# toprakdeviren/gpu-bpe

Hardware: AMD Instinct MI355X
Metric: BPE merges/sec + tokenize GB/s, 1 GiB UTF-8 @ 32K vocab, 1/2/4/8 MI355X (higher is better)
Workload: dtype u16; 1 GPU; headline: 32K-vocab BPE train on 1,073,741,824 B English-like UTF-8 (seed 2, 0.5% 3-byte punctuation), heuristic word boundaries, reference compaction; step = one complete training run (trainer creation + all 32,512 merges) on the HBM-resident corpus; train_bytes=1073741824, target_vocab=32768, parallelism=single

## Files before the change

gpu-bpe_amd/csrc/common.h:

```cpp
#pragma once

#include <hip/hip_runtime.h>
#include <cstdint>
#include <cstdio>
#include <cstdlib>
#include <cstring>
#include <map>
#include <mutex>
#include <string>
#include <type_traits>
#include <unordered_map>
#include <utility>
#include <vector>

#include "../../include/gpubpe.h"

struct GbpePool {
    std::multimap<uint64_t, void*> idle;
    std::unordered_map<void*, uint64_t> busy;
    uint64_t idle_bytes = 0, hits = 0, misses = 0;
};

struct GbpeGrowBuf {
    void* p = nullptr;
// ... 68 lines not shown
        if (p && cap >= n) return hipSuccess;
        GbpeArray nb;
        hipError_t e = nb.reserve(c, n, esz);
        if (e == hipSuccess && p && keep) e = hipMemcpyAsync(nb.p, p, keep * esz, hipMemcpyDeviceToDevice, s);
        if (e == hipSuccess) e = hipStreamSynchronize(s);
        if (e == hipSuccess) *this = std::move(nb);
        return e;
    }
};

int gbpe_set_error(gbpe_ctx* ctx, int code, const char* fmt, ...);

#define GBPE_HIP(ctx, call)                                                              \
    do {                                                                                 \
        hipError_t _e = (call);                                                          \
        if (_e != hipSuccess)                                                            \
            return gbpe_set_error((ctx), _e == hipErrorOutOfMemory ? GBPE_E_OOM           \
                                                                   : GBPE_E_DEVICE,      \
                                  "%s failed: %s (%s:%d)", #call, hipGetErrorString(_e), \
                                  __FILE__, __LINE__);                                   \
    } while (0)

#define GBPE_LAUNCH_CHECK(ctx) GBPE_HIP(ctx, hipGetLastError())

__device__ __forceinline__ uint32_t gbpe_fmix32(uint32_t x) {
    x = (x ^ (x >> 16)) * 0x7feb352du;
    x = (x ^ (x >> 15)) * 0x846ca68bu;
    return x ^ (x >> 16);
}

__host__ __device__ static inline uint64_t gbpe_div_up(uint64_t a, uint64_t b) { return (a + b - 1) / b; }

constexpr const char* kGbpeDebugKeys[] = {
    "lexicon", "lex_check", "rehash", "delta_mt", "zt", "rfl", "rflz", "lxwg", "lxtwo", "pair", "pseg", "prej", "zsmax", "zs32", "poison",
    "encode_slice", "decode_slice", "dec_plain", "me_cs", "htime", "ptrace", "rtime",
};

inline long gbpe_debug_knob(const char* key, long def) {
    const char* e = getenv("GBPE_DEBUG");
    if (!e) return def;
    const size_t kl = strlen(key);
    for (const char* p = e; *p;) {
        if (!strncmp(p, key, kl) && p[kl] == '=') return strtol(p + kl + 1, nullptr, 10);
        const char* c = strchr(p, ',');
        if (!c) break;
        p = c + 1;
    }
    return def;
}

inline std::string gbpe_debug_unknown() {
    const char* e = getenv("GBPE_DEBUG");
    for (const char* p = e ? e : ""; *p;) {
        const size_t el = strcspn(p, ","), kl = strcspn(p, ",=");
        bool ok = el == 0;
        for (const char* k : kGbpeDebugKeys) ok = ok || (kl < el && strlen(k) == kl && !strncmp(p, k, kl));
        if (!ok) return std::string(p, kl ? kl : el);
        p += el + (p[el] == ',');
    }
    return "";
}

int gbpe_pretok_gpt4_launch(gbpe_ctx* ctx, const uint8_t* d_bytes, uint64_t n, uint8_t* d_ws);
int gbpe_pretok_gpt4_docs_launch(gbpe_ctx* ctx, const uint8_t* d_bytes, uint64_t n, const uint8_t* d_flags, uint8_t* d_ws);
int gbpe_pretok_cl100k_launch(gbpe_ctx* ctx, const uint8_t* d_bytes, uint64_t n, const uint8_t* d_flags, uint8_t* d_ws);
int gbpe_pretok_o200k_launch(gbpe_ctx* ctx, const uint8_t* d_bytes, uint64_t n, const uint8_t* d_flags, uint8_t* d_ws);
constexpr uint32_t GBPE_DOC_BAD_ORDER = 1u, GBPE_DOC_BAD_FIRST = 2u, GBPE_DOC_BAD_LAST = 4u;
// ... 9 lines not shown
```

gpu-bpe_amd/csrc/lexicon.h:

```cpp

constexpr uint32_t LX_LIT = 0x80000000u;
constexpr uint32_t LX_LONG = 0x40000000u;
constexpr uint32_t LX_LMAX = 64;
constexpr int LX_WPT = 16;
constexpr int LX_LT = 2048;
constexpr uint32_t LX_PROBES = 4096;

template <typename S>
__device__ __forceinline__ bool lx_is_start(uint32_t prev, uint32_t cur, bool first) {
    return first || (cur & Sym<S>::WS) || !(cur & Sym<S>::TM) || !(prev & Sym<S>::TM);
}

template <typename S>
__global__ __launch_bounds__(TPB) void k_lx_count(const S* __restrict__ x, uint32_t len, uint32_t* __restrict__ tilecnt) {
    __shared__ uint32_t s[TPB / 64];
    const uint64_t base = (uint64_t)blockIdx.x * TILE;
    uint32_t c = 0;
#pragma unroll 4
    for (int k = 0; k < EPT; ++k) {
        const uint64_t i = base + (uint64_t)k * TPB + threadIdx.x;
        if (i < len) c += lx_is_start<S>(i ? (uint32_t)x[i - 1] : 0u, (uint32_t)x[i], i == 0) ? 1u : 0u;
    }
    c = wave_sum_u32(c);
    if ((threadIdx.x & 63) == 0) s[threadIdx.x >> 6] = c;
    __syncthreads();
    if (threadIdx.x == 0) {
        uint32_t t = 0;
        for (int w = 0; w < TPB / 64; ++w) t += s[w];
        tilecnt[blockIdx.x] = t;
    }
}

template <typename S>
__global__ __launch_bounds__(TPB) void k_lx_wpos(const S* __restrict__ x, uint32_t len, const uint32_t* __restrict__ tpre,
                                                 const uint64_t* __restrict__ tblk, uint32_t* __restrict__ wpos) {
    __shared__ uint32_t pre[EPT * (TPB / 64)];
    const int lane = threadIdx.x & 63, wid = threadIdx.x >> 6;
    const uint64_t base = (uint64_t)blockIdx.x * TILE;
    uint32_t f = 0;
#pragma unroll 4
    for (int k = 0; k < EPT; ++k) {
        const uint64_t i = base + (uint64_t)k * TPB + threadIdx.x;
        const bool st = i < len && lx_is_start<S>(i ? (uint32_t)x[i - 1] : 0u, (uint32_t)x[i], i == 0);
        f |= (st ? 1u : 0u) << k;
        const unsigned long long m = __ballot(st);
        if (lane == 0) pre[k * (TPB / 64) + wid] = (uint32_t)__popcll(m);
    }
    __syncthreads();
    if (threadIdx.x == 0) {
        uint32_t run = tpre[blockIdx.x] + (uint32_t)tblk[blockIdx.x / SCAN_BLK];
        for (int q = 0; q < EPT * (TPB / 64); ++q) {
            const uint32_t v = pre[q];
            pre[q] = run;
            run += v;
        }
    }
    __syncthreads();
    const unsigned long long lt = (1ull << lane) - 1ull;
    for (int k = 0; k < EPT; ++k) {
        const bool st = (f >> k) & 1u;
        const unsigned long long m = __ballot(st);
        if (st) wpos[pre[k * (TPB / 64) + wid] + (uint32_t)__popcll(m & lt)] = (uint32_t)(base + (uint64_t)k * TPB + threadIdx.x);
    }
}

template <typename S>
__device__ __forceinline__ unsigned long long lx_hash(const S* __restrict__ x, uint32_t s, uint32_t L) {
    unsigned long long h = 0x9E3779B97F4A7C15ull ^ (unsigned long long)L;
    for (uint32_t i0 = 0; i0 < L; i0 += 8) {
        uint32_t v[8];
#pragma unroll
        for (int k = 0; k < 8; ++k) v[k] = i0 + k < L ? (uint32_t)x[s + i0 + k] : 0u;
#pragma unroll
        for (int k = 0; k < 8; ++k) {
            if (i0 + k >= L) break;
            h ^= (unsigned long long)v[k];
            h *= 0x100000001B3ull;
            h ^= h >> 29;
        }
    }
    h ^= h >> 33;
    h *= 0xff51afd7ed558ccdull;
    h ^= h >> 33;
    h *= 0xc4ceb9fe1a85ec53ull;
    h ^= h >> 33;
    return h ? h : 1ull;
}

__device__ __forceinline__ uint32_t lx_home(unsigned long long h, uint32_t mask) { return (uint32_t)(h ^ (h >> 32)) & mask; }

struct alignas(16) LxSlot {
    unsigned long long key;
    uint32_t rep;
    uint32_t cnt;
};

__device__ __forceinline__ uint32_t lx_slice(uint32_t P) { return P >= (1u << 20) ? P >> 8 : (P < 4096u ? P : 4096u); }
__device__ __forceinline__ uint32_t lx_next(uint32_t slot, uint32_t sm) { return (slot & ~sm) | ((slot + 1u) & sm); }
__device__ __forceinline__ uint32_t lx_bucket(unsigned long long h, uint32_t P) {
    return lx_home(h, P - 1) / lx_slice(P);
}

__device__ bool lx_insert(LxSlot* __restrict__ wt, uint32_t P, unsigned long long h, uint32_t rep, uint32_t c,
                          uint32_t maxp = LX_PROBES) {
    const uint32_t sm = lx_slice(P) - 1u;
    uint32_t slot = lx_home(h, P - 1);
    if (maxp > sm + 1u) maxp = sm + 1u;
    for (uint32_t p = 0; p < maxp; ++p, slot = lx_next(slot, sm)) {
        unsigned long long k = wt[slot].key;
        if (k == 0ull) {
            k = atomicCAS(&wt[slot].key, 0ull, h);
            if (k == 0ull) {
                wt[slot].rep = rep;
                atomicAdd(&wt[slot].cnt, c);
                return true;
            }
        }
        if (k == h) {
            atomicAdd(&wt[slot].cnt, c);
            return true;
        }
    }
    return false;
}

__device__ uint4 lx_find(const LxSlot* __restrict__ wt, uint32_t P, unsigned long long h) {
    const uint32_t sm = lx_slice(P) - 1u;
    uint32_t slot = lx_home(h, P - 1);
    for (uint32_t p = 0; p <= sm && p < LX_PROBES; ++p, slot = lx_next(slot, sm)) {
        const uint4 v = *reinterpret_cast<const uint4*>(&wt[slot]);
        const unsigned long long k = (unsigned long long)v.x | ((unsigned long long)v.y << 32);
        if (k == h) return v;
        if (k == 0ull) break;
    }
    return make_uint4(0u, 0u, SP_INV, SP_INV);
}

template <typename S, int BT = TPB, int LT = LX_LT>
__global__ __launch_bounds__(BT) void k_lx_hash(const S* __restrict__ x, uint32_t len, const uint32_t* __restrict__ wpos,
                                                 uint32_t nw, LxSlot* __restrict__ wtab,
                                                 uint32_t P, uint32_t* __restrict__ otmp, uint32_t* __restrict__ longs,
                                                 uint32_t* __restrict__ ctr, const uint32_t* __restrict__ wmul,
                                                 uint32_t maxp, uint32_t wpt, LxSlot* __restrict__ rec = nullptr,
                                                 uint32_t* __restrict__ bmeta = nullptr, uint32_t nbk = 0,
                                                 uint32_t nwg = 0) {
    __shared__ unsigned long long lk[LT];
    __shared__ uint32_t lc[LT], lr[LT];
    for (int i = threadIdx.x; i < LT; i += BT) {
        lk[i] = 0ull;
        lc[i] = 0u;
    }
    __syncthreads();
    const uint64_t j0 = (uint64_t)blockIdx.x * BT * wpt;
    for (uint32_t q = 0; q < wpt; ++q) {
        const uint64_t j = j0 + (uint64_t)q * BT + threadIdx.x;
        if (j >= nw) break;
        const uint32_t s = wpos[j], e = j + 1 < nw ? wpos[j + 1] : len, L = e - s;
        const uint32_t v0 = x[s];
        if (!(v0 & Sym<S>::TM)) {
            otmp[j] = LX_LIT | v0;
            continue;
        }
        if (L > LX_LMAX) {
            const uint32_t li = atomicAdd(&ctr[0], 1u);
            longs[li] = (uint32_t)j;
            otmp[j] = LX_LONG | li;
            continue;
        }
        otmp[j] = 0u;
        const uint32_t wt = wmul ? wmul[s] : 1u;
        const unsigned long long h = lx_hash<S>(x, s, L);
        uint32_t slot = lx_home(h, LT - 1);
        bool done = false;
        for (int p = 0; p < 32 && !done; ++p, slot = (slot + 1) & (LT - 1)) {
            const unsigned long long o = atomicCAS(&lk[slot], 0ull, h);
            if (o == 0ull) {
                lr[slot] = (uint32_t)j;
                atomicAdd(&lc[slot], wt);
                done = true;
            } else if (o == h) {
                atomicAdd(&lc[slot], wt);
                done = true;
            }
        }
        if (!done && !lx_insert(wtab, P, h, (uint32_t)j, wt, maxp)) ctr[1] = 1u;
    }
    __syncthreads();
    constexpr int FL = LT / BT;
    if (rec) {
        __shared__ uint32_t s_bc[256], s_bo[256], s_ws[BT / 64];
        for (uint32_t i = threadIdx.x; i < 256; i += BT) s_bc[i] = 0u;
        __syncthreads();
        unsigned long long fk[FL];
        uint32_t bk[FL], rk[FL];
#pragma unroll
        for (int q = 0; q < FL; ++q) {
            fk[q] = lk[threadIdx.x + q * BT];
            bk[q] = fk[q] ? lx_bucket(fk[q], P) : 0u;
            rk[q] = fk[q] ? atomicAdd(&s_bc[bk[q]], 1u) : 0u;
        }
        __syncthreads();
        {
            const uint32_t v = threadIdx.x < nbk ? s_bc[threadIdx.x] : 0u;
            const uint32_t incl = wave_scan_incl_u32(v);
// ... 7 lines not shown
                bmeta[(uint64_t)nwg * nbk + (uint64_t)blockIdx.x * nbk + threadIdx.x] = v;
            }
        }
        __syncthreads();
        LxSlot* r = rec + (uint64_t)blockIdx.x * LT;
#pragma unroll
        for (int q = 0; q < FL; ++q) {
            if (!fk[q]) continue;
            const int i = threadIdx.x + q * BT;
            *reinterpret_cast<uint4*>(&r[s_bo[bk[q]] + rk[q]]) =
                make_uint4((uint32_t)fk[q], (uint32_t)(fk[q] >> 32), lr[i], lc[i]);
        }
        return;
    }
    if (__hip_atomic_load(&ctr[1], __ATOMIC_RELAXED, __HIP_MEMORY_SCOPE_AGENT)) return;
    unsigned long long fk[FL], hk[FL];
    uint32_t fs[FL];
#pragma unroll
    for (int q = 0; q < FL; ++q) {
        fk[q] = lk[threadIdx.x + q * BT];
        fs[q] = lx_home(fk[q], P - 1);
        hk[q] = fk[q] ? wtab[fs[q]].key : 0ull;
    }
    bool home[FL];
#pragma unroll
    for (int q = 0; q < FL; ++q) {
        const int i = threadIdx.x + q * BT;
        home[q] = fk[q] && hk[q] == fk[q];
        if (fk[q] && !home[q] && !lx_insert(wtab, P, fk[q], lr[i], lc[i], maxp)) ctr[1] = 1u;
    }
#pragma unroll
    for (int q = 0; q < FL; ++q)
        if (home[q]) atomicAdd(&wtab[fs[q]].cnt, lc[threadIdx.x + q * BT]);
}

constexpr int FOLD_T = 1024, FOLD_LT = 8192, FOLD_B = 8, FOLD_R = 8;
__global__ __launch_bounds__(FOLD_T) void k_lx_fold(const LxSlot* __restrict__ rec, const uint32_t* __restrict__ bmeta,
                                                    uint32_t nwg, uint32_t nbk, LxSlot* __restrict__ wtab, uint32_t P,
                                                    uint32_t* __restrict__ ctr, uint32_t maxp, uint32_t rstride) {
    __shared__ unsigned long long fk[FOLD_LT];
    __shared__ uint32_t fc[FOLD_LT], fr[FOLD_LT];
    if (__hip_atomic_load(&ctr[1], __ATOMIC_RELAXED, __HIP_MEMORY_SCOPE_AGENT)) return;
    for (int i = threadIdx.x; i < FOLD_LT; i += FOLD_T) {
        fk[i] = 0ull;
        fc[i] = 0u;
    }
    __syncthreads();
    const uint32_t b = blockIdx.x;
    bool fail = false;
    for (uint32_t w0 = threadIdx.x; w0 < nwg; w0 += FOLD_T * FOLD_B) {
        uint32_t st[FOLD_B], n[FOLD_B];
#pragma unroll
        for (int k = 0; k < FOLD_B; ++k) {
            const uint32_t w = w0 + (uint32_t)k * FOLD_T;
            st[k] = w < nwg ? bmeta[(uint64_t)w * nbk + b] : 0u;
            n[k] = w < nwg ? bmeta[(uint64_t)nwg * nbk + (uint64_t)w * nbk + b] : 0u;
        }
#pragma unroll 1
        for (int k = 0; k < FOLD_B; ++k) {
            const uint4* r = reinterpret_cast<const uint4*>(rec + (uint64_t)(w0 + (uint32_t)k * FOLD_T) * rstride + st[k]);
            for (uint32_t i0 = 0; i0 < n[k]; i0 += FOLD_R) {
                uint4 v[FOLD_R];
#pragma unroll
                for (int q = 0; q < FOLD_R; ++q) v[q] = i0 + q < n[k] ? r[i0 + q] : make_uint4(0u, 0u, 0u, 0u);
#pragma unroll
                for (int q = 0; q < FOLD_R; ++q) {
// ... 12 lines not shown
                    if (!done && !lx_insert(wtab, P, h, v[q].z, v[q].w, maxp)) fail = true;
                }
            }
        }
    }
    __syncthreads();
    for (int i = threadIdx.x; i < FOLD_LT; i += FOLD_T)
        if (fk[i] && !lx_insert(wtab, P, fk[i], fr[i], fc[i], maxp)) fail = true;
    if (fail) ctr[1] = 1u;
}

constexpr uint32_t LX_TB = TPB * 16;

__device__ __forceinline__ uint64_t lx_tslot(uint32_t k) { return (uint64_t)blockIdx.x * LX_TB + (uint64_t)k * TPB + threadIdx.x; }

__global__ __launch_bounds__(TPB) void k_lx_tabcount(const LxSlot* __restrict__ wt, uint32_t P, uint32_t* __restrict__ cnt) {
    __shared__ uint32_t s[TPB / 64];
    uint32_t c = 0;
#pragma unroll
    for (int k = 0; k < 16; ++k) {
        const uint64_t i = lx_tslot(k);
        c += (i < P && wt[i].key) ? 1u : 0u;
    }
    c = wave_sum_u32(c);
    if ((threadIdx.x & 63) == 0) s[threadIdx.x >> 6] = c;
    __syncthreads();
    if (threadIdx.x == 0) {
        uint32_t t = 0;
        for (int w = 0; w < TPB / 64; ++w) t += s[w];
        cnt[blockIdx.x] = t;
    }
}

__device__ __forceinline__ uint32_t lx_wlen(const uint32_t* __restrict__ wpos, uint32_t nw, uint32_t len, uint32_t j) {
    return (j + 1 < nw ? wpos[j + 1] : len) - wpos[j];
}

__global__ __launch_bounds__(TPB) void k_lx_tabuid(LxSlot* __restrict__ wt, uint32_t P, const uint32_t* __restrict__ bpre,
                                                   const uint64_t* __restrict__ bblk, const uint32_t* __restrict__ wpos,
                                                   uint32_t nw, uint32_t len, uint32_t* __restrict__ usz,
                                                   uint32_t* __restrict__ umul, uint32_t* __restrict__ urep) {
    __shared__ uint32_t s[TPB / 64];
    const int lane = threadIdx.x & 63, wid = threadIdx.x >> 6;
    uint32_t occ = 0;
    uint2 v[16];
#pragma unroll
    for (int k = 0; k < 16; ++k) {
        const uint64_t i = lx_tslot(k);
        const uint4 e = i < P ? *reinterpret_cast<const uint4*>(&wt[i]) : make_uint4(0u, 0u, 0u, 0u);
        v[k] = make_uint2(e.z, e.w);
        occ |= ((e.x | e.y) ? 1u : 0u) << k;
    }
    const uint32_t c = (uint32_t)__popc(occ);
    const uint32_t incl = wave_scan_incl_u32(c);
    if (lane == 63) s[wid] = incl;
    __syncthreads();
    uint32_t u = bpre[blockIdx.x] + (uint32_t)bblk[blockIdx.x / SCAN_BLK] + incl - c;
    for (int w = 0; w < wid; ++w) u += s[w];
#pragma unroll
    for (int k = 0; k < 16; ++k) {
        if (!((occ >> k) & 1u)) continue;
        usz[u] = lx_wlen(wpos, nw, len, v[k].x) + 1u;
        umul[u] = v[k].y;
        urep[u] = wpos[v[k].x];
        wt[lx_tslot(k)].cnt = u;
        ++u;
    }
}

__global__ void k_lx_longs(const uint32_t* __restrict__ longs, const uint32_t* __restrict__ ctr, uint32_t nshort,
                           const uint32_t* __restrict__ wpos, uint32_t nw, uint32_t len, uint32_t* __restrict__ usz,
                           uint32_t* __restrict__ umul, uint32_t* __restrict__ urep,
                           const uint32_t* __restrict__ wmul = nullptr) {
    const uint32_t i = blockIdx.x * blockDim.x + threadIdx.x;
    if (i >= ctr[0]) return;
    const uint32_t j = longs[i];
    usz[nshort + i] = lx_wlen(wpos, nw, len, j) + 1u;
    umul[nshort + i] = wmul ? wmul[wpos[j]] : 1u;
    urep[nshort + i] = wpos[j];
}

template <typename S>
__global__ void k_lx_fill(const S* __restrict__ x, const uint32_t* __restrict__ urep, const uint32_t* __restrict__ usz,
                          const uint32_t* __restrict__ umul, const uint32_t* __restrict__ upre,
                          const uint64_t* __restrict__ ublk, uint32_t nu, S* __restrict__ store, uint32_t* __restrict__ mul) {
    const uint32_t u = blockIdx.x * blockDim.x + threadIdx.x;
    if (u >= nu) return;
    const uint32_t off = upre[u] + (uint32_t)ublk[u / SCAN_BLK], L = usz[u] - 1u, r = urep[u], m = umul[u];
    for (uint32_t i = 0; i < L; ++i) {
        store[off + i] = x[r + i];
        if (mul) mul[off + i] = m;
    }
    store[off + L] = (S)0;
    if (mul) mul[off + L] = 0u;
}

__global__ void k_lx_secstart(const uint32_t* __restrict__ upre, const uint64_t* __restrict__ ublk, uint32_t nu,
                              uint32_t SEC, uint32_t sbase, uint32_t uid_base, uint32_t* __restrict__ starts,
                              uint32_t* __restrict__ w0) {
    const uint32_t u = blockIdx.x * blockDim.x + threadIdx.x;
    if (u >= nu) return;
    const uint32_t o = upre[u] + (uint32_t)ublk[u / SCAN_BLK], k = o / SEC;
    const bool first = u == 0 || (upre[u - 1] + (uint32_t)ublk[(u - 1) / SCAN_BLK]) / SEC != k;
    if (first) {
        starts[k] = sbase + o;
        w0[k] = uid_base + u;
    }
}

template <typename S>
__global__ void k_lx_occ(const S* __restrict__ x, const uint32_t* __restrict__ wpos, uint32_t nw, uint32_t len,
                         const uint32_t* __restrict__ otmp, const LxSlot* __restrict__ wt,
                         uint32_t P, const S* __restrict__ rstore, const uint32_t* __restrict__ upre,
                         const uint64_t* __restrict__ ublk,
                         const uint32_t* __restrict__ usz, uint32_t nshort, uint32_t uid_base, uint32_t* __restrict__ occ,
                         uint32_t* __restrict__ ctr) {
    const uint64_t j = (uint64_t)blockIdx.x * blockDim.x + threadIdx.x;
    if (j >= nw) return;
    const uint32_t o = otmp[j];
    if (o & LX_LIT) {
        occ[j] = o;
        return;
    }
    if (o & LX_LONG) {
        occ[j] = uid_base + nshort + (o & ~LX_LONG);
        return;
    }
    const uint32_t s = wpos[j], L = lx_wlen(wpos, nw, len, (uint32_t)j);
    const uint4 e = lx_find(wt, P, lx_hash<S>(x, s, L));
    bool ok = (e.x | e.y) != 0u;
    uint32_t u = 0;
    if (ok) {
        u = e.w;
        ok = usz[u] == L + 1u;
        const S* r = rstore + upre[u] + ublk[u / SCAN_BLK];
        for (uint32_t i0 = 0; ok && i0 < L; i0 += 8) {
            uint32_t va[8], vb[8];
#pragma unroll
            for (int k = 0; k < 8; ++k) {
                va[k] = i0 + k < L ? (uint32_t)r[i0 + k] : 0u;
                vb[k] = i0 + k < L ? (uint32_t)x[s + i0 + k] : 0u;
            }
#pragma unroll
            for (int k = 0; k < 8; ++k) ok = ok && va[k] == vb[k];
        }
    }
    if (!ok) ctr[1] = 1u;
    occ[j] = uid_base + u;
}


template <typename S>
__global__ __launch_bounds__(TPB) void k_lx_wordpos(const S* __restrict__ store, const uint2* __restrict__ sec,
                                                    uint32_t nsec, const uint32_t* __restrict__ w0,
                                                    uint32_t* __restrict__ coff, uint32_t* __restrict__ clen) {
    const uint32_t k = blockIdx.x * (TPB / 64) + (threadIdx.x >> 6);
    const int lane = threadIdx.x & 63;
    if (k >= nsec) return;
    const uint2 e = sec[k];
    if (!e.y) return;
    uint32_t uid = w0[k], cs = e.x;
    const unsigned long long lt = (1ull << lane) - 1ull;
    for (uint32_t c0 = 0; c0 < e.y; c0 += 64) {
        const uint32_t i = e.x + c0 + (uint32_t)lane;
        const bool sep = c0 + (uint32_t)lane < e.y && store[i] == (S)0;
        const unsigned long long m = __ballot(sep);
        if (sep) {
            const unsigned long long below = m & lt;
            const uint32_t st0 = below ? e.x + c0 + (uint32_t)(63 - __clzll((long long)below)) + 1u : cs;
            const uint32_t u = uid + (uint32_t)__popcll(below);
            coff[u] = st0;
            clen[u] = i - st0;
        }
        uid += (uint32_t)__popcll(m);
        if (m) cs = e.x + c0 + (uint32_t)(63 - __clzll((long long)m)) + 1u;
    }
}

__global__ void k_lx_olen(const uint32_t* __restrict__ occ, uint64_t nocc, const uint32_t* __restrict__ clen,
                          uint32_t* __restrict__ olen, uint32_t nu = 0xFFFFFFFFu, uint32_t* __restrict__ bad = nullptr) {
    const uint64_t j = (uint64_t)blockIdx.x * blockDim.x + threadIdx.x;
// ... 28 lines not shown
```

gpu-bpe_amd/csrc/trainer.h:

```cpp
#pragma once

#include <cmath>

#include "train_dev.h"
#include <chrono>
#include "sparse.h"




struct gbpe_trainer {
    gbpe_ctx* ctx = nullptr;
    bool u16 = true;
    uint32_t bps = 2;
    uint64_t n0 = 0, cap_syms = 0;
    uint64_t n_prev0 = 0;
    uint32_t next_id0 = 256;
    GbpeArray<void> buf[2];
    int cur = 0;
    uint64_t n = 0;
    uint32_t needed = 0, done = 0;
    bool stop = false;
    uint32_t flags = 0, batch = GBPE_BATCH_SIZE;
    GbpeArray<DevState> st;
// ... 20 lines not shown
    GbpeArray<uint2> sec;
    GbpeArray<uint32_t> sp_loc;
    GbpeArray<uint64_t> sp_blk;
    GbpeArray<uint32_t> bits;
    GbpeArray<uint32_t> sig;
    uint64_t sp_age = 0;
    uint64_t sp_bits_age = 0;
    uint32_t W = 0;
    GbpeArray<void> zbuf[2];
    GbpeArray<void> wtmp;
    int zcur = 0;
    GbpeArray<DevState> zst;
    GbpeArray<DevState, true> h_zst;
    GbpeArray<uint32_t> d_u32;
    GbpeArray<uint64_t> part;
    GbpeArray<uint2> zdr_out;
    GbpeArray<uint32_t> zdr_offs, zdr_flag;
    uint32_t zdr_ntile = 0;
    GbpeArray<uint32_t> zseg;
    uint32_t table_grows = 0;
    GbpeArray<uint64_t> wg_bytes;
    uint32_t delta_mt = 2048;
    double ms_sparse = 0, ms_dense = 0;
    double ms_body = 0;
    double ms_create = 0;
    uint64_t dense_bytes = 0;
    uint32_t g_refresh = 0;
    uint64_t sp_merges = 0, sp_sectors = 0, sp_zone = 0;
    uint32_t sp_enters = 0, sp_exits = 0;
    uint32_t sp_cooldown = 0;
    GbpeArray<uint32_t> d_bhist;
    uint32_t lx_wg = 16384;
    bool lx_two = true;
    uint32_t lx_resize = 0;
    uint32_t sp_zt = 5;
    uint32_t refresh_late = 64;
    uint32_t refresh_late_z = 16384;
    bool rehash_on = true;
    uint32_t body_cap = 256;
    bool pair_on = true;
    double pair_rate = 0.5;
    uint64_t pair_done = 0;
    bool pair16_on = true;
    uint32_t zseg_max = NSEG_MAX;
    uint32_t zseg32 = 1;
    uint32_t pair_prej = 0;
    uint32_t ptrace = 0;
    GbpeArray<uint32_t> d_clog;
    GbpeArray<uint32_t, true> h_clog;
    FILE* trace = nullptr;
    uint32_t htime = 0;
    double ht_enq = 0, ht_wait = 0, ht_enq_late = 0, ht_wait_late = 0, ht_pre = 0, ht_post = 0, ht_out = 0;
    double ht_shrink = 0, ht_filters = 0, ht_grow = 0;
    uint64_t ht_nshrink = 0, ht_nfilters = 0;
    std::chrono::steady_clock::time_point ht_last{};
    uint64_t ht_steps = 0, ht_steps_late = 0, ht_merges_late = 0;
    bool lex = false;
    bool lex_on = true;
    bool lex_only = false;
    GbpeArray<void> lx_store;
    GbpeArray<uint32_t> lx_mul;
    uint64_t lx_len = 0;
    GbpeArray<uint32_t> lx_occ;
    uint64_t lx_nocc = 0;
    GbpeArray<uint32_t> lx_w0;
    uint32_t lx_nuid = 0;
// ... 478 lines not shown
    uint64_t Pfull = 4096;
    while (Pfull < 2ull * nw && Pfull < (1ull << 27)) Pfull <<= 1;
    const uint64_t nbbf = gbpe_div_up(Pfull, LX_TB);
    const auto wpt_of = [&](uint64_t nh) {
        return (uint32_t)std::max<uint64_t>(LX_WPT, gbpe_div_up(nh, (uint64_t)TPB * t->lx_wg));
    };
    constexpr uint32_t LX2_T = 1024, LX2_LT = 8192, LX2_WPT = 16;
    const uint64_t nwg_max = gbpe_div_up(nw, (uint64_t)LX2_T * LX2_WPT);
    const bool two = t->lx_two && nw >= (1u << 20);
    const uint64_t need = 9ull * (nw + 64) * 4 + Pfull * 16 + (nbbf + 64) * 4 +
                          2 * (nbbf / SCAN_BLK + (uint64_t)nw / SCAN_BLK + 8) * 8 + 32 * 256 +
                          (two ? nwg_max * LX2_LT * sizeof(LxSlot) + 2 * nwg_max * 256 * 4 + 1024 : 0);
    TR_HIP(t, t->lx_tmp.reserve(t->ctx, need));
    int rc = GBPE_OK;
    LxCarve c{(char*)t->lx_tmp.p};
    lp.wpos = c.take<uint32_t>(nw + 1);
    uint32_t* otmp = c.take<uint32_t>(nw + 1);
    uint32_t* longs = c.take<uint32_t>(nw + 1);
    lp.usz = c.take<uint32_t>(nw + 1);
    lp.umul = c.take<uint32_t>(nw + 1);
    lp.urep = c.take<uint32_t>(nw + 1);
    lp.occ = c.take<uint32_t>(nw + 1);
    auto* wtab = c.take<LxSlot>(Pfull);
    uint32_t* bc = c.take<uint32_t>(nbbf);
    uint64_t* bb = c.take<uint64_t>(nbbf / SCAN_BLK + 4);
    lp.ublk = c.take<uint64_t>((uint64_t)nw / SCAN_BLK + 4);
    uint32_t* ctr = c.take<uint32_t>(8);
    LxSlot* rec = two ? c.take<LxSlot>(nwg_max * LX2_LT) : nullptr;
    uint32_t* bmeta = two ? c.take<uint32_t>(2 * nwg_max * 256) : nullptr;
    hipLaunchKernelGGL(k_lx_wpos<S>, dim3((uint32_t)ntiles), dim3(TPB), 0, s, seg, len, (const uint32_t*)tc,
                       (const uint64_t*)tb, lp.wpos);
    uint32_t h[4] = {0, 0, 0, 0};
    uint64_t nshort = 0;
    auto hash_pass = [&](uint64_t P, uint32_t nh) -> int {
        const uint64_t nbb = gbpe_div_up(P, LX_TB);
        TR_HIP(t, hipMemsetAsync(wtab, 0, P * sizeof(LxSlot), s));
        TR_HIP(t, hipMemsetAsync(ctr, 0, 32, s));
        if (nh) {
            const uint32_t maxp = P < Pfull ? 256u : LX_PROBES;
            const uint32_t nwg2 = (uint32_t)gbpe_div_up(nh, (uint64_t)LX2_T * LX2_WPT);
            if (two && P >= (1ull << 20) && nh >= (1u << 20) && nwg2 <= nwg_max) {
                hipLaunchKernelGGL((k_lx_hash<S, LX2_T, LX2_LT>), dim3(nwg2), dim3(LX2_T), 0, s, seg, len,
                                   (const uint32_t*)lp.wpos, nh, wtab, (uint32_t)P, otmp, longs, ctr, wmul, maxp, LX2_WPT,
                                   rec, bmeta, 256u, nwg2);
                hipLaunchKernelGGL(k_lx_fold, dim3(256), dim3(FOLD_T), 0, s, (const LxSlot*)rec, (const uint32_t*)bmeta,
                                   nwg2, 256u, wtab, (uint32_t)P, ctr, maxp, LX2_LT);
            } else {
                const uint32_t wpt = wpt_of(nh);
                hipLaunchKernelGGL(k_lx_hash<S>, dim3((uint32_t)gbpe_div_up(nh, (uint64_t)TPB * wpt)), dim3(TPB), 0, s, seg,
                                   len, (const uint32_t*)lp.wpos, nh, wtab, (uint32_t)P, otmp, longs, ctr, wmul, maxp, wpt);
            }
        }
        hipLaunchKernelGGL(k_lx_tabcount, dim3((uint32_t)nbb), dim3(TPB), 0, s, (const LxSlot*)wtab, (uint32_t)P, bc);
        lx_scan(s, bc, nbb, bb);
        GBPE_LAUNCH_CHECK(t->ctx);
        TR_HIP(t, hipMemcpyAsync(h, ctr, 8, hipMemcpyDeviceToHost, s));
        TR_HIP(t, hipMemcpyAsync(&nshort, bb + gbpe_div_up(nbb, SCAN_BLK), 8, hipMemcpyDeviceToHost, s));
        TR_HIP(t, hipStreamSynchronize(s));
        return GBPE_OK;
    };
    uint64_t P = Pfull;
    constexpr uint32_t LX_SAMPLE = 1u << 22;
    if (nw > 4u * LX_SAMPLE) {
        rc = hash_pass(2ull * LX_SAMPLE, LX_SAMPLE);
        if (rc != GBPE_OK) return rc;
        if (!h[1]) {
            const double D = (double)(nshort + h[0]) * pow((double)nw / LX_SAMPLE, 0.8);
            uint64_t Pe = 1ull << 20;
            while ((double)Pe < 3.0 * D && Pe < Pfull) Pe <<= 1;
            P = Pe;
        }
    }
    rc = hash_pass(P, nw);
    if (rc != GBPE_OK) return rc;
    if (h[1] && P < Pfull) {
        P = Pfull;
        ++t->lx_resize;
        rc = hash_pass(P, nw);
        if (rc != GBPE_OK) return rc;
    }
    const uint64_t nbb = gbpe_div_up(P, LX_TB);
    if (h[1]) return GBPE_OK;
    lp.nshort = (uint32_t)nshort;
    lp.nlong = h[0];
    lp.nu = lp.nshort + lp.nlong;
    if ((uint64_t)t->lx_nuid + lp.nu >= LX_LONG) return GBPE_OK;
    hipLaunchKernelGGL(k_lx_tabuid, dim3((uint32_t)nbb), dim3(TPB), 0, s, wtab, (uint32_t)P, (const uint32_t*)bc, (const uint64_t*)bb, (const uint32_t*)lp.wpos, nw, len, lp.usz, lp.umul, lp.urep);
    if (lp.nlong)
        hipLaunchKernelGGL(k_lx_longs, dim3((uint32_t)gbpe_div_up(lp.nlong, 256)), dim3(256), 0, s, (const uint32_t*)longs,
                           (const uint32_t*)ctr, lp.nshort, (const uint32_t*)lp.wpos, nw, len, lp.usz, lp.umul, lp.urep,
                           wmul);
    uint32_t* upre = longs;
    TR_HIP(t, hipMemcpyAsync(upre, lp.usz, (uint64_t)lp.nu * 4, hipMemcpyDeviceToDevice, s));
    lx_scan(s, upre, lp.nu, lp.ublk);
    GBPE_LAUNCH_CHECK(t->ctx);
    uint64_t T = 0;
    TR_HIP(t, hipMemcpyAsync(&T, lp.ublk + gbpe_div_up(lp.nu ? lp.nu : 1, SCAN_BLK), 8, hipMemcpyDeviceToHost, s));
    TR_HIP(t, hipStreamSynchronize(s));
    if (fresh && T * 2 > len) return GBPE_OK;
    if (nw) {
        GbpeArray<S> rs_own;
        TR_HIP(t, rs_own.reserve(t->ctx, T + 1));
        S* rstore = rs_own.p;
        if (lp.nu)
            hipLaunchKernelGGL(k_lx_fill<S>, dim3((uint32_t)gbpe_div_up(lp.nu, 256)), dim3(256), 0, s, seg,
                               (const uint32_t*)lp.urep, (const uint32_t*)lp.usz, (const uint32_t*)lp.umul,
                               (const uint32_t*)upre, (const uint64_t*)lp.ublk, lp.nu, rstore, (uint32_t*)nullptr);
        hipLaunchKernelGGL(k_lx_occ<S>, dim3((uint32_t)gbpe_div_up(nw, 256)), dim3(256), 0, s, seg, (const uint32_t*)lp.wpos, nw,
                           len, (const uint32_t*)otmp, (const LxSlot*)wtab, (uint32_t)P, (const S*)rstore,
                           (const uint32_t*)upre, (const uint64_t*)lp.ublk, (const uint32_t*)lp.usz, lp.nshort,
                           t->lx_nuid, lp.occ, ctr);
        GBPE_LAUNCH_CHECK(t->ctx);
        TR_HIP(t, hipMemcpyAsync(h, ctr, 8, hipMemcpyDeviceToHost, s));
        TR_HIP(t, hipStreamSynchronize(s));
        if (h[1]) return GBPE_OK;
    }
    lp.T = (uint32_t)T;
    lp.upre = upre;
    lp.ok = true;
    return GBPE_OK;
}

template <typename S>
int lx_commit(gbpe_trainer* t, LxPlan& lp, const S* seg, bool fresh, bool keep_occ = true) {
    hipStream_t s = t->ctx->stream;
    const uint32_t SEC = SP_SECW;
    const uint64_t sbase = gbpe_div_up(t->lx_len, SEC) * SEC;
    const uint64_t nwin = gbpe_div_up(lp.T ? lp.T : 1, SEC);
    const uint64_t kb = sbase / SEC;
    {
        int rc = sp_reserve(t, kb + nwin, sbase + nwin * SEC, keep_occ ? t->lx_nocc + lp.nw : 0);
        if (rc != GBPE_OK) return rc;
    }
    S* store = (S*)t->lx_store.p;
    if (sbase > t->lx_len) {
        TR_HIP(t, hipMemsetAsync(store + t->lx_len, 0, (sbase - t->lx_len) * sizeof(S), s));
        TR_HIP(t, hipMemsetAsync(t->lx_mul.p + t->lx_len, 0, (sbase - t->lx_len) * 4, s));
    }
    const uint32_t* upre = lp.upre;
    if (lp.nu) {
        hipLaunchKernelGGL(k_lx_fill<S>, dim3((uint32_t)gbpe_div_up(lp.nu, 256)), dim3(256), 0, s, seg,
                           (const uint32_t*)lp.urep, (const uint32_t*)lp.usz, (const uint32_t*)lp.umul, upre,
                           (const uint64_t*)lp.ublk, lp.nu, store + sbase, t->lx_mul.p + sbase);
        TR_HIP(t, hipMemsetAsync(t->sp_loc.p, 0xFF, nwin * 4, s));
// ... 343 lines not shown
    t->lex = false;
    ++t->sp_exits;
    return GBPE_OK;
}

int trainer_config(gbpe_trainer* t, gbpe_ctx* ctx, const gbpe_train_opts* opts) {
    const std::string bad = gbpe_debug_unknown();
    if (!bad.empty()) return gbpe_set_error(ctx, GBPE_E_INVALID, "GBPE_DEBUG: unknown key '%s'", bad.c_str());
    t->ctx = ctx;
    t->flags = opts->flags;
    t->batch = opts->batch_size ? opts->batch_size : GBPE_BATCH_SIZE;
    const uint32_t vocab_size = opts->vocab_size ? opts->vocab_size : 256u;
    const uint32_t next_id = opts->next_token_id ? opts->next_token_id : 256u;
    t->next_id0 = next_id;
    t->needed = opts->target_vocab_size > vocab_size ? opts->target_vocab_size - vocab_size : 0u;
    const uint64_t max_id = (uint64_t)next_id + t->needed;
    t->u16 = max_id <= 0x8000ull;
    t->max_id = (uint32_t)(max_id < 0x10000ull ? max_id : 0x10000ull);
    t->body_cap = (uint32_t)(ctx->num_cu > 0 ? ctx->num_cu : 256);
    t->lex_on = gbpe_debug_knob("lexicon", 1) != 0;
    t->pair_on = gbpe_debug_knob("pair", 1) != 0;
    t->pair16_on = gbpe_debug_knob("pseg", 1) != 0;
    t->pair_prej = (uint32_t)std::max<long>(0, gbpe_debug_knob("prej", 0));
    t->zseg_max = zseg_cap(t->body_cap, gbpe_debug_knob("zsmax", NSEG_MAX));
    t->zseg32 = (uint32_t)gbpe_debug_knob("zs32", t->zseg32);
    t->ptrace = (uint32_t)gbpe_debug_knob("ptrace", 0);
    t->rehash_on = gbpe_debug_knob("rehash", 1) != 0;
    t->delta_mt = (uint32_t)gbpe_debug_knob("delta_mt", t->delta_mt);
    t->sp_zt = (uint32_t)gbpe_debug_knob("zt", t->sp_zt);
    t->refresh_late = (uint32_t)gbpe_debug_knob("rfl", t->refresh_late);
    t->refresh_late_z = (uint32_t)gbpe_debug_knob("rflz", t->refresh_late_z);
    t->lx_wg = (uint32_t)std::max<long>(1, gbpe_debug_knob("lxwg", t->lx_wg));
    t->lx_two = gbpe_debug_knob("lxtwo", 1) != 0;
    t->htime = (uint32_t)gbpe_debug_knob("htime", 0);
    if (t->sp_zt < SP_ZONE_F) t->sp_zt = SP_ZONE_F;
    if (const char* e = getenv("GBPE_SPARSE_TRACE")) {
        t->trace = fopen(e, "w");
        if (t->trace && (t->d_clog.reserve(ctx, (size_t)t->batch * 2) != hipSuccess ||
                         t->h_clog.reserve(ctx, (size_t)t->batch * 2) != hipSuccess))
            t->d_clog.release(), t->h_clog.release();
    }
    t->bps = t->u16 ? 2 : 4;
    return GBPE_OK;
}

int sp_exit_any(gbpe_trainer* t) { return !t->sp ? GBPE_OK : (t->u16 ? sp_exit<uint16_t>(t) : sp_exit<uint32_t>(t)); }

}

struct StateInit {
    const uint32_t* prev;
    uint64_t n_prev;
};
int trainer_create_impl(gbpe_ctx* ctx, const uint8_t* bytes, uint64_t n, const uint8_t* word_starts,
                        int input_on_device, const gbpe_train_opts* opts, uint64_t cap_extra, gbpe_trainer** out,
                        const StateInit* si = nullptr);
```

Baseline: 66570 merges/s.

## Vectorize lexicon word-start scan and occurrence verification with 8-symbol loads

Word-start detection in the count and position kernels now has each thread read 8 contiguous symbols with vector loads and produce an 8-bit start mask. Positions are then placed with a wave inclusive scan plus a bit-iteration loop, replacing the per-element ballot. The occurrence check reads each word's representative offset straight from the hash slot, filled in by a new k_lx_taboff kernel, and compares words in vectorized 8-symbol chunks, dropping the upre, ublk and usz lookups. It also adds a debug hash-bit mask knob and pads the rstore buffer so over-reads stay in bounds, at the cost of one extra kernel launch and less-coalesced strided per-thread loads.

```diff
diff --git a/gpu-bpe_amd/csrc/common.h b/gpu-bpe_amd/csrc/common.h
--- a/gpu-bpe_amd/csrc/common.h
+++ b/gpu-bpe_amd/csrc/common.h
@@ -124,7 +124,7 @@
 __host__ __device__ static inline uint64_t gbpe_div_up(uint64_t a, uint64_t b) { return (a + b - 1) / b; }
 
 constexpr const char* kGbpeDebugKeys[] = {
-    "lexicon", "lex_check", "rehash", "delta_mt", "zt", "rfl", "rflz", "lxwg", "lxtwo", "pair", "pseg", "prej", "zsmax", "zs32", "poison",
+    "lexicon", "lex_check", "rehash", "delta_mt", "zt", "rfl", "rflz", "lxwg", "lxtwo", "lxhbits", "pair", "pseg", "prej", "zsmax", "zs32", "poison",
     "encode_slice", "decode_slice", "dec_plain", "me_cs", "htime", "ptrace", "rtime",
 };
 
diff --git a/gpu-bpe_amd/csrc/lexicon.h b/gpu-bpe_amd/csrc/lexicon.h
--- a/gpu-bpe_amd/csrc/lexicon.h
+++ b/gpu-bpe_amd/csrc/lexicon.h
@@ -12,15 +12,54 @@
 }
 
 template <typename S>
+__device__ __forceinline__ void lx_load8(const S* __restrict__ y, uint32_t s, uint32_t n, uint32_t len, uint32_t (&v)[8]) {
+    if ((uint64_t)s + 8u <= len) {
+        typedef uint32_t V4 __attribute__((ext_vector_type(4)));
+        typedef V4 V4A2 __attribute__((aligned(2)));
+        typedef V4 V4A4 __attribute__((aligned(4)));
+        using V4S = typename std::conditional<sizeof(S) == 2, V4A2, V4A4>::type;
+        constexpr int NV = (int)(8 * sizeof(S) / 16), PV = (int)(16 / sizeof(S));
+#pragma unroll
+        for (int q = 0; q < NV; ++q) {
+            const V4 t = *reinterpret_cast<const V4S*>(y + s + q * PV);
+#pragma unroll
+            for (int k = 0; k < PV; ++k) {
+                const uint32_t d = t[k * (int)sizeof(S) / 4];
+                const uint32_t sym = sizeof(S) == 2 ? (k & 1 ? d >> 16 : d & 0xFFFFu) : d;
+                v[q * PV + k] = (uint32_t)(q * PV + k) < n ? sym : 0u;
+            }
+        }
+    } else {
+#pragma unroll
+        for (int k = 0; k < 8; ++k) v[k] = (uint32_t)k < n ? (uint32_t)y[s + k] : 0u;
+    }
+}
+
+template <typename S>
+__device__ __forceinline__ uint32_t lx_starts8(const S* __restrict__ x, uint32_t len, uint64_t i0) {
+    if (i0 >= len) return 0u;
+    const uint32_t n = len - i0 < 8u ? (uint32_t)(len - i0) : 8u;
+    uint32_t v[8];
+    lx_load8<S>(x, (uint32_t)i0, n, len, v);
+    uint32_t prev = i0 ? (uint32_t)x[i0 - 1] : 0u, m = 0;
+#pragma unroll
+    for (int k = 0; k < 8; ++k) {
+        if ((uint32_t)k < n && lx_is_start<S>(prev, v[k], i0 + k == 0)) m |= 1u << k;
+        prev = v[k];
+    }
+    return m;
+}
+
+static_assert(EPT % 8 == 0, "a thread takes whole 8-symbol vectors of its tile");
+constexpr int LX_VPT = EPT / 8;
+
+template <typename S>
 __global__ __launch_bounds__(TPB) void k_lx_count(const S* __restrict__ x, uint32_t len, uint32_t* __restrict__ tilecnt) {
     __shared__ uint32_t s[TPB / 64];
     const uint64_t base = (uint64_t)blockIdx.x * TILE;
     uint32_t c = 0;
-#pragma unroll 4
-    for (int k = 0; k < EPT; ++k) {
-        const uint64_t i = base + (uint64_t)k * TPB + threadIdx.x;
-        if (i < len) c += lx_is_start<S>(i ? (uint32_t)x[i - 1] : 0u, (uint32_t)x[i], i == 0) ? 1u : 0u;
-    }
+#pragma unroll
+    for (int r = 0; r < LX_VPT; ++r) c += (uint32_t)__popc(lx_starts8<S>(x, len, base + ((uint64_t)r * TPB + threadIdx.x) * 8u));
     c = wave_sum_u32(c);
     if ((threadIdx.x & 63) == 0) s[threadIdx.x >> 6] = c;
     __syncthreads();
@@ -34,43 +73,46 @@
 template <typename S>
 __global__ __launch_bounds__(TPB) void k_lx_wpos(const S* __restrict__ x, uint32_t len, const uint32_t* __restrict__ tpre,
                                                  const uint64_t* __restrict__ tblk, uint32_t* __restrict__ wpos) {
-    __shared__ uint32_t pre[EPT * (TPB / 64)];
+    __shared__ uint32_t pre[LX_VPT * (TPB / 64)];
     const int lane = threadIdx.x & 63, wid = threadIdx.x >> 6;
     const uint64_t base = (uint64_t)blockIdx.x * TILE;
-    uint32_t f = 0;
-#pragma unroll 4
-    for (int k = 0; k < EPT; ++k) {
-        const uint64_t i = base + (uint64_t)k * TPB + threadIdx.x;
-        const bool st = i < len && lx_is_start<S>(i ? (uint32_t)x[i - 1] : 0u, (uint32_t)x[i], i == 0);
-        f |= (st ? 1u : 0u) << k;
-        const unsigned long long m = __ballot(st);
-        if (lane == 0) pre[k * (TPB / 64) + wid] = (uint32_t)__popcll(m);
+    uint32_t m[LX_VPT], before[LX_VPT];
+#pragma unroll
+    for (int r = 0; r < LX_VPT; ++r) {
+        m[r] = lx_starts8<S>(x, len, base + ((uint64_t)r * TPB + threadIdx.x) * 8u);
+        const uint32_t c = (uint32_t)__popc(m[r]), incl = wave_scan_incl_u32(c);
+        before[r] = incl - c;
+        if (lane == 63) pre[r * (TPB / 64) + wid] = incl;
     }
     __syncthreads();
     if (threadIdx.x == 0) {
         uint32_t run = tpre[blockIdx.x] + (uint32_t)tblk[blockIdx.x / SCAN_BLK];
-        for (int q = 0; q < EPT * (TPB / 64); ++q) {
+        for (int q = 0; q < LX_VPT * (TPB / 64); ++q) {
             const uint32_t v = pre[q];
             pre[q] = run;
             run += v;
         }
     }
     __syncthreads();
-    const unsigned long long lt = (1ull << lane) - 1ull;
-    for (int k = 0; k < EPT; ++k) {
-        const bool st = (f >> k) & 1u;
-        const unsigned long long m = __ballot(st);
-        if (st) wpos[pre[k * (TPB / 64) + wid] + (uint32_t)__popcll(m & lt)] = (uint32_t)(base + (uint64_t)k * TPB + threadIdx.x);
-    }
-}
-
-template <typename S>
-__device__ __forceinline__ unsigned long long lx_hash(const S* __restrict__ x, uint32_t s, uint32_t L) {
+#pragma unroll
+    for (int r = 0; r < LX_VPT; ++r) {
+        uint32_t at = pre[r * (TPB / 64) + wid] + before[r];
+        const uint32_t i0 = (uint32_t)(base + ((uint64_t)r * TPB + threadIdx.x) * 8u);
+        for (uint32_t mm = m[r]; mm; mm &= mm - 1u) wpos[at++] = i0 + (uint32_t)__ffs(mm) - 1u;
+    }
+}
+
+template <typename S>
+__device__ __forceinline__ unsigned long long lx_hash(const S* __restrict__ x, uint32_t s, uint32_t L, uint32_t len,
+                                                      unsigned long long hmask, uint32_t (&first)[8]) {
     unsigned long long h = 0x9E3779B97F4A7C15ull ^ (unsigned long long)L;
     for (uint32_t i0 = 0; i0 < L; i0 += 8) {
         uint32_t v[8];
-#pragma unroll
-        for (int k = 0; k < 8; ++k) v[k] = i0 + k < L ? (uint32_t)x[s + i0 + k] : 0u;
+        lx_load8<S>(x, s + i0, L - i0, len, v);
+        if (i0 == 0) {
+#pragma unroll
+            for (int k = 0; k < 8; ++k) first[k] = v[k];
+        }
 #pragma unroll
         for (int k = 0; k < 8; ++k) {
             if (i0 + k >= L) break;
@@ -84,6 +126,7 @@
     h ^= h >> 33;
     h *= 0xc4ceb9fe1a85ec53ull;
     h ^= h >> 33;
+    h &= hmask;
     return h ? h : 1ull;
 }
 
@@ -141,7 +184,8 @@
                                                  uint32_t nw, LxSlot* __restrict__ wtab,
                                                  uint32_t P, uint32_t* __restrict__ otmp, uint32_t* __restrict__ longs,
                                                  uint32_t* __restrict__ ctr, const uint32_t* __restrict__ wmul,
-                                                 uint32_t maxp, uint32_t wpt, LxSlot* __restrict__ rec = nullptr,
+                                                 uint32_t maxp, uint32_t wpt, unsigned long long hmask,
+                                                 LxSlot* __restrict__ rec = nullptr,
                                                  uint32_t* __restrict__ bmeta = nullptr, uint32_t nbk = 0,
                                                  uint32_t nwg = 0) {
     __shared__ unsigned long long lk[LT];
@@ -169,7 +213,8 @@
         }
         otmp[j] = 0u;
         const uint32_t wt = wmul ? wmul[s] : 1u;
-        const unsigned long long h = lx_hash<S>(x, s, L);
+        uint32_t first[8];
+        const unsigned long long h = lx_hash<S>(x, s, L, len, hmask, first);
         uint32_t slot = lx_home(h, LT - 1);
         bool done = false;
         for (int p = 0; p < 32 && !done; ++p, slot = (slot + 1) & (LT - 1)) {
@@ -243,6 +288,10 @@
 #pragma unroll
     for (int q = 0; q < FL; ++q)
         if (home[q]) atomicAdd(&wtab[fs[q]].cnt, lc[threadIdx.x + q * BT]);
+}
+
+__device__ __forceinline__ uint32_t lx_wlen(const uint32_t* __restrict__ wpos, uint32_t nw, uint32_t len, uint32_t j) {
+    return (j + 1 < nw ? wpos[j + 1] : len) - wpos[j];
 }
 
 constexpr int FOLD_T = 1024, FOLD_LT = 8192, FOLD_B = 8, FOLD_R = 8;
@@ -321,10 +370,6 @@
     }
 }
 
-__device__ __forceinline__ uint32_t lx_wlen(const uint32_t* __restrict__ wpos, uint32_t nw, uint32_t len, uint32_t j) {
-    return (j + 1 < nw ? wpos[j + 1] : len) - wpos[j];
-}
-
 __global__ __launch_bounds__(TPB) void k_lx_tabuid(LxSlot* __restrict__ wt, uint32_t P, const uint32_t* __restrict__ bpre,
                                                    const uint64_t* __restrict__ bblk, const uint32_t* __restrict__ wpos,
                                                    uint32_t nw, uint32_t len, uint32_t* __restrict__ usz,
@@ -354,6 +399,17 @@
         urep[u] = wpos[v[k].x];
         wt[lx_tslot(k)].cnt = u;
         ++u;
+    }
+}
+
+__global__ __launch_bounds__(TPB) void k_lx_taboff(LxSlot* __restrict__ wt, uint32_t P, const uint32_t* __restrict__ upre,
+                                                   const uint64_t* __restrict__ ublk) {
+#pragma unroll
+    for (int k = 0; k < 16; ++k) {
+        const uint64_t i = lx_tslot(k);
+        if (i >= P || !wt[i].key) continue;
+        const uint32_t u = wt[i].cnt;
+        wt[i].rep = upre[u] + (uint32_t)ublk[u / SCAN_BLK];
     }
 }
 
@@ -400,10 +456,8 @@
 template <typename S>
 __global__ void k_lx_occ(const S* __restrict__ x, const uint32_t* __restrict__ wpos, uint32_t nw, uint32_t len,
                          const uint32_t* __restrict__ otmp, const LxSlot* __restrict__ wt,
-                         uint32_t P, const S* __restrict__ rstore, const uint32_t* __restrict__ upre,
-                         const uint64_t* __restrict__ ublk,
-                         const uint32_t* __restrict__ usz, uint32_t nshort, uint32_t uid_base, uint32_t* __restrict__ occ,
-                         uint32_t* __restrict__ ctr) {
+                         uint32_t P, const S* __restrict__ rstore, uint32_t rlen, uint32_t nshort, uint32_t uid_base,
+                         uint32_t* __restrict__ occ, uint32_t* __restrict__ ctr, unsigned long long hmask) {
     const uint64_t j = (uint64_t)blockIdx.x * blockDim.x + threadIdx.x;
     if (j >= nw) return;
     const uint32_t o = otmp[j];
@@ -416,26 +470,22 @@
         return;
     }
     const uint32_t s = wpos[j], L = lx_wlen(wpos, nw, len, (uint32_t)j);
-    const uint4 e = lx_find(wt, P, lx_hash<S>(x, s, L));
+    uint32_t w[8], r[8];
+    const uint4 e = lx_find(wt, P, lx_hash<S>(x, s, L, len, hmask, w));
     bool ok = (e.x | e.y) != 0u;
-    uint32_t u = 0;
     if (ok) {
-        u = e.w;
-        ok = usz[u] == L + 1u;
-        const S* r = rstore + upre[u] + ublk[u / SCAN_BLK];
-        for (uint32_t i0 = 0; ok && i0 < L; i0 += 8) {
-            uint32_t va[8], vb[8];
-#pragma unroll
-            for (int k = 0; k < 8; ++k) {
-                va[k] = i0 + k < L ? (uint32_t)r[i0 + k] : 0u;
-                vb[k] = i0 + k < L ? (uint32_t)x[s + i0 + k] : 0u;
-            }
-#pragma unroll
-            for (int k = 0; k < 8; ++k) ok = ok && va[k] == vb[k];
+        lx_load8<S>(rstore, e.z, L + 1u, rlen, r);
+#pragma unroll
+        for (int k = 0; k < 8; ++k) ok = ok && w[k] == r[k];
+        for (uint32_t i0 = 8; ok && i0 <= L; i0 += 8) {
+            lx_load8<S>(x, s + i0, L - i0, len, w);
+            lx_load8<S>(rstore, e.z + i0, L + 1u - i0, rlen, r);
+#pragma unroll
+            for (int k = 0; k < 8; ++k) ok = ok && w[k] == r[k];
         }
     }
     if (!ok) ctr[1] = 1u;
-    occ[j] = uid_base + u;
+    occ[j] = uid_base + ((e.x | e.y) ? e.w : 0u);
 }
 
 
diff --git a/gpu-bpe_amd/csrc/trainer.h b/gpu-bpe_amd/csrc/trainer.h
--- a/gpu-bpe_amd/csrc/trainer.h
+++ b/gpu-bpe_amd/csrc/trainer.h
@@ -76,6 +76,7 @@
     GbpeArray<uint32_t> d_bhist;
     uint32_t lx_wg = 16384;
     bool lx_two = true;
+    unsigned long long lx_hmask = ~0ull;
     uint32_t lx_resize = 0;
     uint32_t sp_zt = 5;
     uint32_t refresh_late = 64;
@@ -620,6 +621,7 @@
                        (const uint64_t*)tb, lp.wpos);
     uint32_t h[4] = {0, 0, 0, 0};
     uint64_t nshort = 0;
+    const unsigned long long hmask = t->lx_hmask;
     auto hash_pass = [&](uint64_t P, uint32_t nh) -> int {
         const uint64_t nbb = gbpe_div_up(P, LX_TB);
         TR_HIP(t, hipMemsetAsync(wtab, 0, P * sizeof(LxSlot), s));
@@ -630,13 +632,14 @@
             if (two && P >= (1ull << 20) && nh >= (1u << 20) && nwg2 <= nwg_max) {
                 hipLaunchKernelGGL((k_lx_hash<S, LX2_T, LX2_LT>), dim3(nwg2), dim3(LX2_T), 0, s, seg, len,
                                    (const uint32_t*)lp.wpos, nh, wtab, (uint32_t)P, otmp, longs, ctr, wmul, maxp, LX2_WPT,
-                                   rec, bmeta, 256u, nwg2);
+                                   hmask, rec, bmeta, 256u, nwg2);
                 hipLaunchKernelGGL(k_lx_fold, dim3(256), dim3(FOLD_T), 0, s, (const LxSlot*)rec, (const uint32_t*)bmeta,
                                    nwg2, 256u, wtab, (uint32_t)P, ctr, maxp, LX2_LT);
             } else {
                 const uint32_t wpt = wpt_of(nh);
                 hipLaunchKernelGGL(k_lx_hash<S>, dim3((uint32_t)gbpe_div_up(nh, (uint64_t)TPB * wpt)), dim3(TPB), 0, s, seg,
-                                   len, (const uint32_t*)lp.wpos, nh, wtab, (uint32_t)P, otmp, longs, ctr, wmul, maxp, wpt);
+                                   len, (const uint32_t*)lp.wpos, nh, wtab, (uint32_t)P, otmp, longs, ctr, wmul, maxp, wpt,
+                                   hmask);
             }
         }
         hipLaunchKernelGGL(k_lx_tabcount, dim3((uint32_t)nbb), dim3(TPB), 0, s, (const LxSlot*)wtab, (uint32_t)P, bc);
@@ -688,16 +691,18 @@
     if (fresh && T * 2 > len) return GBPE_OK;
     if (nw) {
         GbpeArray<S> rs_own;
-        TR_HIP(t, rs_own.reserve(t->ctx, T + 1));
+        TR_HIP(t, rs_own.reserve(t->ctx, T + LX_LMAX + 8));
         S* rstore = rs_own.p;
         if (lp.nu)
             hipLaunchKernelGGL(k_lx_fill<S>, dim3((uint32_t)gbpe_div_up(lp.nu, 256)), dim3(256), 0, s, seg,
                                (const uint32_t*)lp.urep, (const uint32_t*)lp.usz, (const uint32_t*)lp.umul,
                                (const uint32_t*)upre, (const uint64_t*)lp.ublk, lp.nu, rstore, (uint32_t*)nullptr);
+        if (lp.nshort)
+            hipLaunchKernelGGL(k_lx_taboff, dim3((uint32_t)nbb), dim3(TPB), 0, s, wtab, (uint32_t)P, (const uint32_t*)upre,
+                               (const uint64_t*)lp.ublk);
         hipLaunchKernelGGL(k_lx_occ<S>, dim3((uint32_t)gbpe_div_up(nw, 256)), dim3(256), 0, s, seg, (const uint32_t*)lp.wpos, nw,
                            len, (const uint32_t*)otmp, (const LxSlot*)wtab, (uint32_t)P, (const S*)rstore,
-                           (const uint32_t*)upre, (const uint64_t*)lp.ublk, (const uint32_t*)lp.usz, lp.nshort,
-                           t->lx_nuid, lp.occ, ctr);
+                           (uint32_t)(T + LX_LMAX + 8), lp.nshort, t->lx_nuid, lp.occ, ctr, hmask);
         GBPE_LAUNCH_CHECK(t->ctx);
         TR_HIP(t, hipMemcpyAsync(h, ctr, 8, hipMemcpyDeviceToHost, s));
         TR_HIP(t, hipStreamSynchronize(s));
@@ -1107,6 +1112,10 @@
     t->refresh_late_z = (uint32_t)gbpe_debug_knob("rflz", t->refresh_late_z);
     t->lx_wg = (uint32_t)std::max<long>(1, gbpe_debug_knob("lxwg", t->lx_wg));
     t->lx_two = gbpe_debug_knob("lxtwo", 1) != 0;
+    {
+        const long hb = gbpe_debug_knob("lxhbits", 64);
+        t->lx_hmask = hb >= 64 ? ~0ull : hb <= 0 ? 0ull : (1ull << hb) - 1ull;
+    }
     t->htime = (uint32_t)gbpe_debug_knob("htime", 0);
     if (t->sp_zt < SP_ZONE_F) t->sp_zt = SP_ZONE_F;
     if (const char* e = getenv("GBPE_SPARSE_TRACE")) {
```

Measured after the change: 67130 merges/s (median of 6 runs). No clear change (+0.8%).
